# 0xC0000054/avif-format

Hardware: NVIDIA H100
Metric: Gpixels/s (higher is better)
Workload: dtype f32

## Files before the change

avif-format_b200/csrc/kernels_fast_flat.cu:

```cuda
#include "kernels_fast_common.cuh"
#include "table_staging.cuh"
#include "../../include/avifgpu.h"

namespace avifgpu
{

using namespace avifpix;
using namespace fastenc;
using namespace staging;
using avifmath::LibmTables;

namespace
{

#ifndef AVIF_FLAT_WARPS
#define AVIF_FLAT_WARPS 28
#endif
constexpr int kFlatWarps = AVIF_FLAT_WARPS;
constexpr int kFlatThreads = kFlatWarps * 32;
constexpr int kRowSegmentBytes = kTilePixels * 12;
constexpr int kStageBytesPerWarp = 2 * kRowSegmentBytes;
constexpr int kRowSegmentWords = kRowSegmentBytes / 4;
constexpr int kSharedBarriers = 256;
constexpr int kTableBarrierSlot = kSharedBarriers / 8 - 1;
static_assert(kFlatWarps <= kTableBarrierSlot, "the warps' barriers and the table's share kSharedBarriers");
constexpr int kSharedLimit = 227 * 1024;
__host__ __device__ constexpr int FlatFixedBytes() { return kSharedLibm + kSharedBarriers + kFlatWarps * kStageBytesPerWarp; }

struct FlatSchedule
{
    int32_t tilesX, tileRows, warpCount;
    int32_t segments, items;
    int32_t segmentRows, longSegments;
    int32_t lastColumnBytes;
    int32_t unpairedTileRow;
    int32_t scatter;
};

__device__ __forceinline__ bool ElectOne()
{
    uint32_t elected;
    asm volatile("{ .reg .pred p; elect.sync _|p, 0xffffffff; selp.u32 %0, 1, 0, p; }" : "=r"(elected));
    return elected != 0;
}

template <int CURVE, int XS, int YS, int TWO_LEVEL, int INTERLEAVED>
__global__ void __launch_bounds__(kFlatThreads, 1) EncodeRgbF32FlatKernel(const FastEncodeParams p, const FlatSchedule schedule)
{
    constexpr bool kCompact = TWO_LEVEL >= 2;
    constexpr int kCompactShift = TWO_LEVEL == 3 ? 14 : 0;
    extern __shared__ __align__(128) uint8_t sharedBytes[];
    uint64_t* libmStorage = reinterpret_cast<uint64_t*>(sharedBytes);
    uint64_t* barriers = reinterpret_cast<uint64_t*>(sharedBytes + kSharedLibm);
    uint8_t* stageAll = sharedBytes + kSharedLibm + kSharedBarriers;
    uint2* flatEntries = reinterpret_cast<uint2*>(sharedBytes + FlatFixedBytes());
    uint32_t* compactEntries = reinterpret_cast<uint32_t*>(sharedBytes + FlatFixedBytes());
    const uint32_t* firstBits = compactEntries + ((p.table.flatCount + 3) & ~3);
    uint2* octaves = reinterpret_cast<uint2*>(sharedBytes + FlatFixedBytes());
    uint32_t* bucketWords = reinterpret_cast<uint32_t*>(sharedBytes + FlatFixedBytes() + 2048);

    const int lane = threadIdx.x & 31;
    const int warpInBlock = __shfl_sync(0xffffffffu, static_cast<int>(threadIdx.x >> 5), 0);
    const uint32_t barrier = SharedAddress(barriers + warpInBlock);
    uint32_t* stage = reinterpret_cast<uint32_t*>(stageAll + warpInBlock * kStageBytesPerWarp);
    const uint32_t stageAddress = SharedAddress(stage);
    const uint32_t* myStage = stage + lane * 12;

    const int tilesX = schedule.tilesX;
    const int warpCount = schedule.warpCount;
    const int firstItem = schedule.scatter ? warpInBlock * static_cast<int>(gridDim.x) + static_cast<int>(blockIdx.x) : static_cast<int>(blockIdx.x) * kFlatWarps + warpInBlock;
    constexpr int kChromaRowsPerTile = YS ? 1 : 2;
    constexpr int kChromaTileBytes = XS ? kTilePixels : 2 * kTilePixels;

    auto itemRows = [&](int item, int& column, int& rowBegin, int& rowEnd)
    {
        const int segment = item / tilesX;
        column = item - segment * tilesX;
        rowBegin = segment * schedule.segmentRows + min(segment, schedule.longSegments);
        rowEnd = rowBegin + schedule.segmentRows + (segment < schedule.longSegments ? 1 : 0);
    };
    auto fetchTile = [&](int row, uint32_t bytes, int64_t offset)
    {
        const bool second = row != schedule.unpairedTileRow;
        const uint8_t* source = p.rows + offset;
        BarrierExpect(barrier, second ? 2u * bytes : bytes);
        BulkCopyToShared(stageAddress, source, bytes, barrier);
        if (second)
        {
            BulkCopyToShared(stageAddress + kRowSegmentBytes, source + p.rowStride, bytes, barrier);
        }
    };
    auto columnBytes = [&](int column) { return column == tilesX - 1 ? static_cast<uint32_t>(schedule.lastColumnBytes) : static_cast<uint32_t>(kRowSegmentBytes); };
    auto sourceOffsetOf = [&](int row, int column) { return static_cast<int64_t>(row) * 2 * p.rowStride + static_cast<int64_t>(column) * kRowSegmentBytes; };

    if (kCompact && threadIdx.x == 0)
    {
        BeginTableImageCopy(p.table, compactEntries, barriers + kTableBarrierSlot);
    }
    if (ElectOne())
    {
        BarrierInit(barrier, 1);
        BarrierInitFence();
        if (firstItem < schedule.items)
        {
            int column, rowBegin, rowEnd;
            itemRows(firstItem, column, rowBegin, rowEnd);
            if (rowBegin < rowEnd)
            {
                fetchTile(rowBegin, columnBytes(column), sourceOffsetOf(rowBegin, column));
            }
        }
    }

    const LibmTables t = avifmath::StageLibmTables(libmStorage, threadIdx.x, blockDim.x);
    if (kCompact)
    {
    }
    else if (TWO_LEVEL)
    {
        for (int i = threadIdx.x; i < 256; i += blockDim.x)
        {
            octaves[i] = p.table.octaves[i];
        }
        for (int i = threadIdx.x; i < p.table.bucketCount; i += blockDim.x)
        {
            bucketWords[i] = p.table.buckets[i];
        }
    }
    else
    {
        const uint4* source = reinterpret_cast<const uint4*>(p.table.flat);
        uint4* target = reinterpret_cast<uint4*>(flatEntries);
        const int pairs = (p.table.flatCount + 1) / 2;
#pragma unroll 8
        for (int i = threadIdx.x; i < pairs; i += blockDim.x)
        {
            target[i] = __ldg(source + i);
        }
    }
    __syncthreads();
    if (kCompact)
    {
        WaitTableImage(barriers + kTableBarrierSlot);
    }

    const uint32_t flatShift = p.table.flatShift;
    const int32_t negativeLow = -static_cast<int32_t>(p.table.flatLow);
    const int32_t span = static_cast<int32_t>(p.table.flatHigh - p.table.flatLow);
    const uint32_t bandStrideLog2 = p.table.bandStrideLog2;
    const uint32_t* __restrict__ bandBits = p.table.bandBits;
    const uint32_t compactTopShift = 32u - flatShift;
    const uint32_t compactCodeMask = p.table.compactCodeMask;
    const uint32_t compactMagic = p.table.compactMagic;
    uint32_t parity = 0;

#pragma unroll 1
    for (int item = firstItem; item < schedule.items; item += warpCount)
    {
        int column, rowBegin, rowEnd;
        itemRows(item, column, rowBegin, rowEnd);
        if (item != firstItem && rowBegin < rowEnd && ElectOne())
        {
            fetchTile(rowBegin, columnBytes(column), sourceOffsetOf(rowBegin, column));
        }
        const uint32_t tileBytes = columnBytes(column);
        const bool laneActive = column * kTilePixels + lane * 4 < p.width;
        int64_t sourceOffset = sourceOffsetOf(rowBegin, column);
        uint8_t* yPointer = p.planeY + static_cast<int64_t>(rowBegin) * 2 * p.strideY +
                            (INTERLEAVED ? static_cast<int64_t>(column) * (6 * kTilePixels) + lane * 24 : static_cast<int64_t>(column) * (2 * kTilePixels) + lane * 8);
        uint8_t* cbPointer = p.planeCb + static_cast<int64_t>(rowBegin) * kChromaRowsPerTile * p.strideCb + static_cast<int64_t>(column) * kChromaTileBytes + lane * (XS ? 4 : 8);
        uint8_t* crPointer = p.planeCr + static_cast<int64_t>(rowBegin) * kChromaRowsPerTile * p.strideCr + static_cast<int64_t>(column) * kChromaTileBytes + lane * (XS ? 4 : 8);

#pragma unroll 1
    for (int tileRow = rowBegin; tileRow < rowEnd; ++tileRow)
    {
        const bool secondRow = tileRow != schedule.unpairedTileRow;
        sourceOffset += 2 * p.rowStride;

        BarrierWait(barrier, parity);
        parity ^= 1u;

        float codeF[kValuesPerLane];
        uint32_t bandMask = 0;
        int32_t largest = 0;
#pragma unroll
        for (int q = 0; q < 6; ++q)
        {
            const uint4 w = *reinterpret_cast<const uint4*>(myStage + (q / 3) * kRowSegmentWords + (q % 3) * 4);
            const uint32_t bits[4] = { w.x, w.y, w.z, w.w };
#pragma unroll
            for (int e = 0; e < 4; ++e)
            {
                const int j = 4 * q + e;
                bool inBand;
                if (kCompact)
                {
                    uint32_t entry;
                    codeF[j] = LookupCurveCompact<kCompactShift>(bits[e], compactEntries, flatShift, negativeLow, span, compactTopShift, compactCodeMask,
                                                                 compactMagic, inBand, entry);
                }
                else if (TWO_LEVEL)
                {
                    codeF[j] = CodeToFloat(LookupCurveCode(bits[e], octaves, bucketWords, inBand));
                }
                else
                {
                    codeF[j] = LookupCurveFlat(bits[e], flatEntries, flatShift, negativeLow, span, inBand);
                }
                asm("{ .reg .pred p; setp.ne.u32 p, %1, 0; @p or.b32 %0, %0, %2; }" : "+r"(bandMask) : "r"(static_cast<uint32_t>(inBand)), "r"(1u << j));
            }
            if (TWO_LEVEL != 1)
            {
                largest = max(largest, __vimax3_s32(static_cast<int32_t>(w.x), static_cast<int32_t>(w.y), static_cast<int32_t>(w.z)));
                largest = max(largest, static_cast<int32_t>(w.w));
            }
        }

        auto stagedBits = [&](int j) { return myStage[j + (j >= 12 ? kRowSegmentWords - 12 : 0)]; };
        uint32_t lowerMask = 0;
        if (kCompact)
        {
            uint32_t pending = bandMask;
            while (pending != 0)
            {
                uint32_t word[2] = { 0xffffffffu, 0xffffffffu }, index[2] = { 0u, 0u }, sampleBit[2] = { 0u, 0u };
#pragma unroll
                for (int u = 0; u < 2; ++u)
                {
                    if (pending != 0)
                    {
                        const int j = __ffs(static_cast<int>(pending)) - 1;
                        pending &= pending - 1;
                        const uint32_t bits = stagedBits(j);
                        const int32_t bucket = __viaddmin_s32_relu(static_cast<int32_t>(bits) >> flatShift, negativeLow, span);
                        const uint32_t entry = compactEntries[bucket];
                        const uint32_t k = ((entry & compactCodeMask) >> kCompactLenBits) + ((entry >> compactTopShift) != 0 ? 1u : 0u);
                        const uint32_t distance = bits - firstBits[k];
                        if (k != 0 && distance < (1u << bandStrideLog2))
                        {
                            index[u] = (k << bandStrideLog2) + distance;
                            word[u] = __ldg(bandBits + (index[u] >> 5));
                            sampleBit[u] = 1u << j;
                        }
                    }
                }
#pragma unroll
                for (int u = 0; u < 2; ++u)
                {
                    if (((word[u] >> (index[u] & 31u)) & 1u) == 0)
                    {
                        lowerMask |= sampleBit[u];
                    }
                }
            }
        }
        else if (!TWO_LEVEL)
        {
            uint32_t pending = bandMask;
            while (pending != 0)
            {
                const int j0 = __ffs(static_cast<int>(pending)) - 1;
                pending &= pending - 1;
                const uint32_t bits0 = stagedBits(j0);
                bool inBand;
                uint2 entry0;
                LookupCurveFlat(bits0, flatEntries, flatShift, negativeLow, span, inBand, entry0);
                const uint32_t index0 = BandBitIndex(bits0, entry0, bandStrideLog2);
                const uint32_t word0 = __ldg(bandBits + (index0 >> 5));
                uint32_t word1 = 0xffffffffu, index1 = 0, sample1 = 0;
                if (pending != 0)
                {
                    const int j1 = __ffs(static_cast<int>(pending)) - 1;
                    pending &= pending - 1;
                    const uint32_t bits1 = stagedBits(j1);
                    uint2 entry1;
                    LookupCurveFlat(bits1, flatEntries, flatShift, negativeLow, span, inBand, entry1);
                    index1 = BandBitIndex(bits1, entry1, bandStrideLog2);
                    word1 = __ldg(bandBits + (index1 >> 5));
                    sample1 = 1u << j1;
                }
                lowerMask |= (((word0 >> (index0 & 31u)) & 1u) ^ 1u) << j0;
                if (((word1 >> (index1 & 31u)) & 1u) == 0)
                {
                    lowerMask |= sample1;
                }
            }
        }

        if (__any_sync(0xffffffffu, TWO_LEVEL == 1 ? bandMask != 0 : largest > 0x7f7fffff))
        {
            for (int j = 0; j < kValuesPerLane; ++j)
            {
                const uint32_t bits = stagedBits(j);
                if (TWO_LEVEL == 1 ? ((bandMask >> j) & 1u) != 0 : static_cast<int32_t>(bits) > 0x7f7fffff)
                {
                    const float exact = CodeToFloat(ExactCurveCode<CURVE>(__uint_as_float(bits), p.pqMultiplier, p.maxCodeFloat, t));
#pragma unroll
                    for (int slot = 0; slot < kValuesPerLane; ++slot)
                    {
                        if (slot == j)
                        {
                            codeF[slot] = exact;
                        }
                    }
                }
            }
        }

        __syncwarp();
        if (tileRow + 1 < rowEnd && ElectOne())
        {
            fetchTile(tileRow + 1, tileBytes, sourceOffset);
        }

#pragma unroll
        for (int j = 0; j < kValuesPerLane; ++j)
        {
            if (lowerMask & (1u << j))
            {
                codeF[j] -= 1.0f;
            }
        }

        if (laneActive)
        {
            if (INTERLEAVED)
            {
#pragma unroll
                for (int r = 0; r < 2; ++r)
                {
                    if (r == 1 && !secondRow) break;
                    uint32_t words[6];
#pragma unroll
                    for (int w = 0; w < 6; ++w)
                    {
                        words[w] = __float2uint_rz(codeF[12 * r + 2 * w]) | (__float2uint_rz(codeF[12 * r + 2 * w + 1]) << 16);
                    }
                    uint2* target = reinterpret_cast<uint2*>(yPointer + r * p.strideY);
                    __stcs(target, make_uint2(words[0], words[1]));
                    __stcs(target + 1, make_uint2(words[2], words[3]));
                    __stcs(target + 2, make_uint2(words[4], words[5]));
                }
            }
            else
            {
                StoreTile<XS, YS>(p, codeF, yPointer, cbPointer, crPointer, secondRow);
            }
        }
        yPointer += 2 * p.strideY;
        cbPointer += kChromaRowsPerTile * p.strideCb;
        crPointer += kChromaRowsPerTile * p.strideCr;
    }
    }
}

inline size_t TableSharedBytes(const FastEncodeParams& fp, int tableKind)
{
    if (tableKind == 1) return 2048 + static_cast<size_t>(fp.table.bucketCount) * sizeof(uint32_t);
    if (tableKind >= 2) return fp.table.compactImageBytes;
    return static_cast<size_t>((fp.table.flatCount + 1) / 2) * sizeof(uint4);
}

template <int CURVE, int XS, int YS, int TWO_LEVEL, int INTERLEAVED = 0>
cudaError_t LaunchFlatKernel(const FastEncodeParams& fp, int smCount, cudaStream_t stream)
{
    const size_t shared = static_cast<size_t>(FlatFixedBytes()) + TableSharedBytes(fp, TWO_LEVEL);
    static std::atomic<uint64_t> configuredDevices{ 0 };
    {
        const cudaError_t e = AllowDynamicShared(EncodeRgbF32FlatKernel<CURVE, XS, YS, TWO_LEVEL, INTERLEAVED>, kSharedLimit, configuredDevices);
        if (e != cudaSuccess)
        {
            return e;
        }
    }
    const long long tiles = static_cast<long long>((fp.width + kTilePixels - 1) / kTilePixels) * ((fp.rowCount + 1) / 2);
    if (tiles > 0x7fffffffll || shared > static_cast<size_t>(kSharedLimit))
    {
        return cudaErrorInvalidValue;
    }
    long long blocks = (tiles + kFlatWarps - 1) / kFlatWarps;
    if (blocks > smCount)
    {
        blocks = smCount;
    }
    FlatSchedule schedule{};
    schedule.tilesX = (fp.width + kTilePixels - 1) / kTilePixels;
    schedule.tileRows = (fp.rowCount + 1) / 2;
    schedule.warpCount = static_cast<int32_t>(blocks) * kFlatWarps;
    schedule.segments = schedule.warpCount / schedule.tilesX;
    if (schedule.segments < 1) schedule.segments = 1;
    if (schedule.segments > schedule.tileRows) schedule.segments = schedule.tileRows;
    schedule.items = schedule.tilesX * schedule.segments;
    schedule.segmentRows = schedule.tileRows / schedule.segments;
    schedule.longSegments = schedule.tileRows % schedule.segments;
    schedule.lastColumnBytes = (fp.width - (schedule.tilesX - 1) * kTilePixels) * 12;
    schedule.unpairedTileRow = (fp.rowCount & 1) ? fp.rowCount / 2 : -1;
    static const bool scatterOff = []() { const char* v = getenv("AVIFGPU_FLAT_SCATTER"); return v != nullptr && v[0] == '0'; }();
    schedule.scatter = scatterOff ? 0 : 1;
    EncodeRgbF32FlatKernel<CURVE, XS, YS, TWO_LEVEL, INTERLEAVED><<<static_cast<unsigned>(blocks), kFlatThreads, shared, stream>>>(fp, schedule);
    return cudaGetLastError();
}

template <int CURVE, int TWO_LEVEL>
cudaError_t DispatchFlatChroma(const FastEncodeParams& fp, int xs, int ys, int smCount, cudaStream_t stream)
{
    if (xs == 1 && ys == 1) return LaunchFlatKernel<CURVE, 1, 1, TWO_LEVEL>(fp, smCount, stream);
    if (xs == 1) return LaunchFlatKernel<CURVE, 1, 0, TWO_LEVEL>(fp, smCount, stream);
    return LaunchFlatKernel<CURVE, 0, 0, TWO_LEVEL>(fp, smCount, stream);
}

}

static bool FlatTableFits(const FastEncodeParams& fp)
{
    return fp.table.flat != nullptr && fp.table.bandBits != nullptr &&
           static_cast<size_t>(FlatFixedBytes()) + TableSharedBytes(fp, 0) <= static_cast<size_t>(kSharedLimit);
}

static bool CompactTableFits(const FastEncodeParams& fp)
{
    return fp.table.compact != nullptr && fp.table.firstBits != nullptr && fp.table.bandBits != nullptr &&
           static_cast<size_t>(FlatFixedBytes()) + TableSharedBytes(fp, 2) <= static_cast<size_t>(kSharedLimit);
}

static bool TwoLevelTableFits(const FastEncodeParams& fp)
{
    return fp.table.buckets != nullptr && fp.table.octaves != nullptr &&
           static_cast<size_t>(FlatFixedBytes()) + TableSharedBytes(fp, 1) <= static_cast<size_t>(kSharedLimit);
}

bool FlatEncodeApplies(const FastEncodeParams& fp)
{
    return CompactTableFits(fp) || FlatTableFits(fp) || TwoLevelTableFits(fp);
}

cudaError_t LaunchFastEncodeFlatInterleaved(const FastEncodeParams& fp, int curve, int smCount, cudaStream_t stream)
{
    if (CompactTableFits(fp))
    {
        if (curve == kCurveLinearToPQ)
        {
            return fp.table.flatShift == 14 ? LaunchFlatKernel<kCurveLinearToPQ, 0, 0, 3, 1>(fp, smCount, stream) : LaunchFlatKernel<kCurveLinearToPQ, 0, 0, 2, 1>(fp, smCount, stream);
        }
        return LaunchFlatKernel<kCurveLinearToSMPTE428, 0, 0, 2, 1>(fp, smCount, stream);
    }
    if (FlatTableFits(fp))
    {
        if (curve == kCurveLinearToPQ) return LaunchFlatKernel<kCurveLinearToPQ, 0, 0, 0, 1>(fp, smCount, stream);
        return LaunchFlatKernel<kCurveLinearToSMPTE428, 0, 0, 0, 1>(fp, smCount, stream);
    }
    if (curve == kCurveLinearToPQ) return LaunchFlatKernel<kCurveLinearToPQ, 0, 0, 1, 1>(fp, smCount, stream);
    return LaunchFlatKernel<kCurveLinearToSMPTE428, 0, 0, 1, 1>(fp, smCount, stream);
}

cudaError_t LaunchFastEncodeFlat(const FastEncodeParams& fp, int curve, int xs, int ys, int smCount, cudaStream_t stream)
{
    if (CompactTableFits(fp) && !fp.preferWideEntries)
    {
        if (curve == kCurveLinearToPQ)
        {
            return fp.table.flatShift == 14 ? DispatchFlatChroma<kCurveLinearToPQ, 3>(fp, xs, ys, smCount, stream) : DispatchFlatChroma<kCurveLinearToPQ, 2>(fp, xs, ys, smCount, stream);
        }
        return DispatchFlatChroma<kCurveLinearToSMPTE428, 2>(fp, xs, ys, smCount, stream);
    }
    if (FlatTableFits(fp))
    {
        if (curve == kCurveLinearToPQ) return DispatchFlatChroma<kCurveLinearToPQ, 0>(fp, xs, ys, smCount, stream);
        return DispatchFlatChroma<kCurveLinearToSMPTE428, 0>(fp, xs, ys, smCount, stream);
    }
    if (curve == kCurveLinearToPQ) return DispatchFlatChroma<kCurveLinearToPQ, 1>(fp, xs, ys, smCount, stream);
    return DispatchFlatChroma<kCurveLinearToSMPTE428, 1>(fp, xs, ys, smCount, stream);
}

}
```

avif-format_b200/csrc/table_staging.cuh:

```cuda
#ifndef AVIFGPU_TABLE_STAGING_CUH
#define AVIFGPU_TABLE_STAGING_CUH

#include "curve_tables.h"

#include <stdint.h>

namespace avifgpu
{
namespace staging
{

constexpr uint32_t kTableCopyChunk = 16384;

__device__ __forceinline__ uint32_t SharedAddress(const void* pointer) { return static_cast<uint32_t>(__cvta_generic_to_shared(pointer)); }

__device__ __forceinline__ void BarrierInit(uint32_t barrier, uint32_t arrivals)
{
    asm volatile("mbarrier.init.shared::cta.b64 [%0], %1;" ::"r"(barrier), "r"(arrivals) : "memory");
}

__device__ __forceinline__ void BarrierInitFence() { asm volatile("fence.mbarrier_init.release.cluster;" ::: "memory"); }

__device__ __forceinline__ void BarrierExpect(uint32_t barrier, uint32_t bytes)
{
    asm volatile("mbarrier.arrive.expect_tx.shared::cta.b64 _, [%0], %1;" ::"r"(barrier), "r"(bytes) : "memory");
}

__device__ __forceinline__ void BulkCopyToShared(uint32_t target, const void* source, uint32_t bytes, uint32_t barrier)
{
    asm volatile("cp.async.bulk.shared::cluster.global.mbarrier::complete_tx::bytes [%0], [%1], %2, [%3];" ::"r"(target), "l"(source), "r"(bytes),
                 "r"(barrier)
                 : "memory");
}

__device__ __forceinline__ void BarrierWait(uint32_t barrier, uint32_t parity)
{
    asm volatile(
        "{\n"
        ".reg .pred done;\n"
        "WAIT_LOOP:\n"
        "mbarrier.try_wait.parity.shared::cta.b64 done, [%0], %1;\n"
        "@done bra WAIT_DONE;\n"
        "bra WAIT_LOOP;\n"
        "WAIT_DONE:\n"
        "}\n" ::"r"(barrier),
        "r"(parity)
        : "memory");
}

__device__ __forceinline__ void BeginTableImageCopy(const CurveTableView& table, void* sharedImage, uint64_t* barrierStorage)
{
    const uint32_t barrier = SharedAddress(barrierStorage);
    BarrierInit(barrier, 1);
    BarrierInitFence();
    const uint32_t imageBytes = table.compactImageBytes;
    BarrierExpect(barrier, imageBytes);
    const uint32_t target = SharedAddress(sharedImage);
    const uint8_t* source = reinterpret_cast<const uint8_t*>(table.compact);
    for (uint32_t offset = 0; offset < imageBytes; offset += kTableCopyChunk)
    {
        BulkCopyToShared(target + offset, source + offset, min(kTableCopyChunk, imageBytes - offset), barrier);
    }
}

__device__ __forceinline__ void WaitTableImage(uint64_t* barrierStorage) { BarrierWait(SharedAddress(barrierStorage), 0); }

}
}

#endif
```

Measured before the change: 185.8.

## Replace segmented flat schedule with grid-strided tile walk and L2 prefetch

The flat encode kernel no longer splits rows into per-column segments that each warp walks vertically. Each warp now strides through tiles in raster order by the total warp count. It also issues an L2 bulk prefetch for its second tile and loads the compact table with an evict_last cache policy so the table stays resident in L2. The intent is better load balance, interleaved DRAM access across warps and less startup latency, at the cost of losing vertical locality and recomputing output pointers per tile. Profiling probe scripts that compare the encode against copy-throughput ceilings are also added.

```diff
diff --git a/avif-format_b200/csrc/kernels_fast_flat.cu b/avif-format_b200/csrc/kernels_fast_flat.cu
--- a/avif-format_b200/csrc/kernels_fast_flat.cu
+++ b/avif-format_b200/csrc/kernels_fast_flat.cu
@@ -29,12 +29,10 @@
 
 struct FlatSchedule
 {
-    int32_t tilesX, tileRows, warpCount;
-    int32_t segments, items;
-    int32_t segmentRows, longSegments;
+    int32_t tilesX, tileRows;
+    int32_t stepRows, stepColumns;
     int32_t lastColumnBytes;
     int32_t unpairedTileRow;
-    int32_t scatter;
 };
 
 __device__ __forceinline__ bool ElectOne()
@@ -67,22 +65,21 @@
     const uint32_t* myStage = stage + lane * 12;
 
     const int tilesX = schedule.tilesX;
-    const int warpCount = schedule.warpCount;
-    const int firstItem = schedule.scatter ? warpInBlock * static_cast<int>(gridDim.x) + static_cast<int>(blockIdx.x) : static_cast<int>(blockIdx.x) * kFlatWarps + warpInBlock;
+    const int tileRows = schedule.tileRows;
     constexpr int kChromaRowsPerTile = YS ? 1 : 2;
     constexpr int kChromaTileBytes = XS ? kTilePixels : 2 * kTilePixels;
 
-    auto itemRows = [&](int item, int& column, int& rowBegin, int& rowEnd)
-    {
-        const int segment = item / tilesX;
-        column = item - segment * tilesX;
-        rowBegin = segment * schedule.segmentRows + min(segment, schedule.longSegments);
-        rowEnd = rowBegin + schedule.segmentRows + (segment < schedule.longSegments ? 1 : 0);
-    };
-    auto fetchTile = [&](int row, uint32_t bytes, int64_t offset)
+    int tileRow, column;
+    {
+        const int first = warpInBlock * static_cast<int>(gridDim.x) + static_cast<int>(blockIdx.x);
+        tileRow = first / tilesX;
+        column = first - tileRow * tilesX;
+    }
+    auto fetchTile = [&](int row, int col)
     {
         const bool second = row != schedule.unpairedTileRow;
-        const uint8_t* source = p.rows + offset;
+        const uint32_t bytes = col == tilesX - 1 ? static_cast<uint32_t>(schedule.lastColumnBytes) : static_cast<uint32_t>(kRowSegmentBytes);
+        const uint8_t* source = p.rows + static_cast<int64_t>(row) * 2 * p.rowStride + static_cast<int64_t>(col) * kRowSegmentBytes;
         BarrierExpect(barrier, second ? 2u * bytes : bytes);
         BulkCopyToShared(stageAddress, source, bytes, barrier);
         if (second)
@@ -90,25 +87,37 @@
             BulkCopyToShared(stageAddress + kRowSegmentBytes, source + p.rowStride, bytes, barrier);
         }
     };
-    auto columnBytes = [&](int column) { return column == tilesX - 1 ? static_cast<uint32_t>(schedule.lastColumnBytes) : static_cast<uint32_t>(kRowSegmentBytes); };
-    auto sourceOffsetOf = [&](int row, int column) { return static_cast<int64_t>(row) * 2 * p.rowStride + static_cast<int64_t>(column) * kRowSegmentBytes; };
+    auto prefetchSecondTile = [&]()
+    {
+        int row = tileRow + schedule.stepRows, col = column + schedule.stepColumns;
+        if (col >= tilesX)
+        {
+            col -= tilesX;
+            ++row;
+        }
+        if (row < tileRows)
+        {
+            const uint32_t bytes = col == tilesX - 1 ? static_cast<uint32_t>(schedule.lastColumnBytes) : static_cast<uint32_t>(kRowSegmentBytes);
+            const uint8_t* source = p.rows + static_cast<int64_t>(row) * 2 * p.rowStride + static_cast<int64_t>(col) * kRowSegmentBytes;
+            asm volatile("cp.async.bulk.prefetch.L2.global [%0], %1;" ::"l"(source), "r"(bytes) : "memory");
+            if (row != schedule.unpairedTileRow)
+            {
+                asm volatile("cp.async.bulk.prefetch.L2.global [%0], %1;" ::"l"(source + p.rowStride), "r"(bytes) : "memory");
+            }
+        }
+    };
 
     if (kCompact && threadIdx.x == 0)
     {
-        BeginTableImageCopy(p.table, compactEntries, barriers + kTableBarrierSlot);
+        BeginTableImageCopy(p.table, compactEntries, barriers + kTableBarrierSlot, true);
     }
     if (ElectOne())
     {
         BarrierInit(barrier, 1);
         BarrierInitFence();
-        if (firstItem < schedule.items)
-        {
-            int column, rowBegin, rowEnd;
-            itemRows(firstItem, column, rowBegin, rowEnd);
-            if (rowBegin < rowEnd)
-            {
-                fetchTile(rowBegin, columnBytes(column), sourceOffsetOf(rowBegin, column));
-            }
+        if (tileRow < tileRows)
+        {
+            fetchTile(tileRow, column);
         }
     }
 
@@ -142,6 +151,10 @@
     if (kCompact)
     {
         WaitTableImage(barriers + kTableBarrierSlot);
+    }
+    if (tileRow < tileRows && ElectOne())
+    {
+        prefetchSecondTile();
     }
 
     const uint32_t flatShift = p.table.flatShift;
@@ -155,27 +168,15 @@
     uint32_t parity = 0;
 
 #pragma unroll 1
-    for (int item = firstItem; item < schedule.items; item += warpCount)
-    {
-        int column, rowBegin, rowEnd;
-        itemRows(item, column, rowBegin, rowEnd);
-        if (item != firstItem && rowBegin < rowEnd && ElectOne())
-        {
-            fetchTile(rowBegin, columnBytes(column), sourceOffsetOf(rowBegin, column));
-        }
-        const uint32_t tileBytes = columnBytes(column);
-        const bool laneActive = column * kTilePixels + lane * 4 < p.width;
-        int64_t sourceOffset = sourceOffsetOf(rowBegin, column);
-        uint8_t* yPointer = p.planeY + static_cast<int64_t>(rowBegin) * 2 * p.strideY +
-                            (INTERLEAVED ? static_cast<int64_t>(column) * (6 * kTilePixels) + lane * 24 : static_cast<int64_t>(column) * (2 * kTilePixels) + lane * 8);
-        uint8_t* cbPointer = p.planeCb + static_cast<int64_t>(rowBegin) * kChromaRowsPerTile * p.strideCb + static_cast<int64_t>(column) * kChromaTileBytes + lane * (XS ? 4 : 8);
-        uint8_t* crPointer = p.planeCr + static_cast<int64_t>(rowBegin) * kChromaRowsPerTile * p.strideCr + static_cast<int64_t>(column) * kChromaTileBytes + lane * (XS ? 4 : 8);
-
-#pragma unroll 1
-    for (int tileRow = rowBegin; tileRow < rowEnd; ++tileRow)
+    while (tileRow < tileRows)
     {
         const bool secondRow = tileRow != schedule.unpairedTileRow;
-        sourceOffset += 2 * p.rowStride;
+        int nextRow = tileRow + schedule.stepRows, nextColumn = column + schedule.stepColumns;
+        if (nextColumn >= tilesX)
+        {
+            nextColumn -= tilesX;
+            ++nextRow;
+        }
 
         BarrierWait(barrier, parity);
         parity ^= 1u;
@@ -308,9 +309,9 @@
         }
 
         __syncwarp();
-        if (tileRow + 1 < rowEnd && ElectOne())
-        {
-            fetchTile(tileRow + 1, tileBytes, sourceOffset);
+        if (nextRow < tileRows && ElectOne())
+        {
+            fetchTile(nextRow, nextColumn);
         }
 
 #pragma unroll
@@ -322,8 +323,12 @@
             }
         }
 
-        if (laneActive)
-        {
+        if (column * kTilePixels + lane * 4 < p.width)
+        {
+            uint8_t* yPointer = p.planeY + static_cast<int64_t>(tileRow) * 2 * p.strideY +
+                                (INTERLEAVED ? static_cast<int64_t>(column) * (6 * kTilePixels) + lane * 24 : static_cast<int64_t>(column) * (2 * kTilePixels) + lane * 8);
+            uint8_t* cbPointer = p.planeCb + static_cast<int64_t>(tileRow) * kChromaRowsPerTile * p.strideCb + static_cast<int64_t>(column) * kChromaTileBytes + lane * (XS ? 4 : 8);
+            uint8_t* crPointer = p.planeCr + static_cast<int64_t>(tileRow) * kChromaRowsPerTile * p.strideCr + static_cast<int64_t>(column) * kChromaTileBytes + lane * (XS ? 4 : 8);
             if (INTERLEAVED)
             {
 #pragma unroll
@@ -347,10 +352,8 @@
                 StoreTile<XS, YS>(p, codeF, yPointer, cbPointer, crPointer, secondRow);
             }
         }
-        yPointer += 2 * p.strideY;
-        cbPointer += kChromaRowsPerTile * p.strideCb;
-        crPointer += kChromaRowsPerTile * p.strideCr;
-    }
+        tileRow = nextRow;
+        column = nextColumn;
     }
 }
 
@@ -386,17 +389,11 @@
     FlatSchedule schedule{};
     schedule.tilesX = (fp.width + kTilePixels - 1) / kTilePixels;
     schedule.tileRows = (fp.rowCount + 1) / 2;
-    schedule.warpCount = static_cast<int32_t>(blocks) * kFlatWarps;
-    schedule.segments = schedule.warpCount / schedule.tilesX;
-    if (schedule.segments < 1) schedule.segments = 1;
-    if (schedule.segments > schedule.tileRows) schedule.segments = schedule.tileRows;
-    schedule.items = schedule.tilesX * schedule.segments;
-    schedule.segmentRows = schedule.tileRows / schedule.segments;
-    schedule.longSegments = schedule.tileRows % schedule.segments;
+    const int32_t warpCount = static_cast<int32_t>(blocks) * kFlatWarps;
+    schedule.stepRows = warpCount / schedule.tilesX;
+    schedule.stepColumns = warpCount % schedule.tilesX;
     schedule.lastColumnBytes = (fp.width - (schedule.tilesX - 1) * kTilePixels) * 12;
     schedule.unpairedTileRow = (fp.rowCount & 1) ? fp.rowCount / 2 : -1;
-    static const bool scatterOff = []() { const char* v = getenv("AVIFGPU_FLAT_SCATTER"); return v != nullptr && v[0] == '0'; }();
-    schedule.scatter = scatterOff ? 0 : 1;
     EncodeRgbF32FlatKernel<CURVE, XS, YS, TWO_LEVEL, INTERLEAVED><<<static_cast<unsigned>(blocks), kFlatThreads, shared, stream>>>(fp, schedule);
     return cudaGetLastError();
 }
diff --git a/avif-format_b200/csrc/table_staging.cuh b/avif-format_b200/csrc/table_staging.cuh
--- a/avif-format_b200/csrc/table_staging.cuh
+++ b/avif-format_b200/csrc/table_staging.cuh
@@ -33,6 +33,20 @@
                  : "memory");
 }
 
+__device__ __forceinline__ uint64_t PolicyEvictLast()
+{
+    uint64_t policy;
+    asm volatile("createpolicy.fractional.L2::evict_last.b64 %0, 1.0;" : "=l"(policy));
+    return policy;
+}
+
+__device__ __forceinline__ void BulkCopyToShared(uint32_t target, const void* source, uint32_t bytes, uint32_t barrier, uint64_t policy)
+{
+    asm volatile("cp.async.bulk.shared::cluster.global.mbarrier::complete_tx::bytes.L2::cache_hint [%0], [%1], %2, [%3], %4;" ::"r"(target),
+                 "l"(source), "r"(bytes), "r"(barrier), "l"(policy)
+                 : "memory");
+}
+
 __device__ __forceinline__ void BarrierWait(uint32_t barrier, uint32_t parity)
 {
     asm volatile(
@@ -48,7 +62,7 @@
         : "memory");
 }
 
-__device__ __forceinline__ void BeginTableImageCopy(const CurveTableView& table, void* sharedImage, uint64_t* barrierStorage)
+__device__ __forceinline__ void BeginTableImageCopy(const CurveTableView& table, void* sharedImage, uint64_t* barrierStorage, bool keepInL2 = false)
 {
     const uint32_t barrier = SharedAddress(barrierStorage);
     BarrierInit(barrier, 1);
@@ -59,7 +73,15 @@
     const uint8_t* source = reinterpret_cast<const uint8_t*>(table.compact);
     for (uint32_t offset = 0; offset < imageBytes; offset += kTableCopyChunk)
     {
-        BulkCopyToShared(target + offset, source + offset, min(kTableCopyChunk, imageBytes - offset), barrier);
+        const uint32_t bytes = min(kTableCopyChunk, imageBytes - offset);
+        if (keepInL2)
+        {
+            BulkCopyToShared(target + offset, source + offset, bytes, barrier, PolicyEvictLast());
+        }
+        else
+        {
+            BulkCopyToShared(target + offset, source + offset, bytes, barrier);
+        }
     }
 }
 
diff --git a/profiles/c2_ceiling_probe.cu b/profiles/c2_ceiling_probe.cu
--- /dev/null
+++ b/profiles/c2_ceiling_probe.cu
@@ -0,0 +1,138 @@
+#include <cuda_runtime.h>
+#include <stdint.h>
+
+namespace
+{
+
+constexpr int kChunkBytes = 3072;
+constexpr int kChunkOut = kChunkBytes / 4;
+constexpr int kMaxStages = 2;
+
+__device__ __forceinline__ uint4 Xor4(uint4 a, uint4 b, uint4 c, uint4 d)
+{
+    return make_uint4(a.x ^ b.x ^ c.x ^ d.x, a.y ^ b.y ^ c.y ^ d.y, a.z ^ b.z ^ c.z ^ d.z, a.w ^ b.w ^ c.w ^ d.w);
+}
+
+__global__ void __launch_bounds__(256) CopyMixLdg(const uint4* __restrict__ in, uint4* __restrict__ out, long long outWords)
+{
+    const int lane = threadIdx.x & 31;
+    const long long warp = (static_cast<long long>(blockIdx.x) * blockDim.x + threadIdx.x) >> 5;
+    const long long warps = (static_cast<long long>(gridDim.x) * blockDim.x) >> 5;
+    for (long long base = warp * 32; base < outWords; base += warps * 32)
+    {
+        const uint4* source = in + base * 4;
+        const uint4 a = __ldcs(source + lane), b = __ldcs(source + 32 + lane), c = __ldcs(source + 64 + lane), d = __ldcs(source + 96 + lane);
+        __stcs(out + base + lane, Xor4(a, b, c, d));
+    }
+}
+
+__device__ __forceinline__ uint32_t SharedAddress(const void* p) { return static_cast<uint32_t>(__cvta_generic_to_shared(p)); }
+
+__device__ __forceinline__ void Fetch(uint32_t target, const void* source, uint32_t barrier)
+{
+    asm volatile("mbarrier.arrive.expect_tx.shared::cta.b64 _, [%0], %1;" ::"r"(barrier), "r"(kChunkBytes) : "memory");
+    asm volatile("cp.async.bulk.shared::cluster.global.mbarrier::complete_tx::bytes [%0], [%1], %2, [%3];" ::"r"(target), "l"(source),
+                 "r"(kChunkBytes), "r"(barrier)
+                 : "memory");
+}
+
+__device__ __forceinline__ void Wait(uint32_t barrier, uint32_t parity)
+{
+    asm volatile("{\n.reg .pred done;\nPROBE_WAIT:\nmbarrier.try_wait.parity.shared::cta.b64 done, [%0], %1;\n@!done bra PROBE_WAIT;\n}\n" ::"r"(barrier),
+                 "r"(parity)
+                 : "memory");
+}
+
+__global__ void CopyMixBulk(const uint8_t* __restrict__ in, uint4* __restrict__ out, int chunks, int stages)
+{
+    extern __shared__ __align__(128) uint8_t shared[];
+    const int lane = threadIdx.x & 31;
+    const int warpInBlock = __shfl_sync(0xffffffffu, static_cast<int>(threadIdx.x >> 5), 0);
+    const int warpsPerBlock = blockDim.x >> 5;
+    uint64_t* barriers = reinterpret_cast<uint64_t*>(shared) + warpInBlock * kMaxStages;
+    uint8_t* stage = shared + 1024 + warpInBlock * kMaxStages * kChunkBytes;
+    const int warps = warpsPerBlock * gridDim.x;
+    const int first = warpInBlock * gridDim.x + blockIdx.x;
+    if (lane == 0)
+    {
+        for (int s = 0; s < stages; ++s)
+        {
+            asm volatile("mbarrier.init.shared::cta.b64 [%0], 1;" ::"r"(SharedAddress(barriers + s)) : "memory");
+        }
+        asm volatile("fence.mbarrier_init.release.cluster;" ::: "memory");
+        for (int s = 0; s < stages; ++s)
+        {
+            const int chunk = first + s * warps;
+            if (chunk < chunks)
+            {
+                Fetch(SharedAddress(stage + s * kChunkBytes), in + static_cast<long long>(chunk) * kChunkBytes, SharedAddress(barriers + s));
+            }
+        }
+    }
+    __syncwarp();
+    int s = 0;
+    uint32_t parity = 0;
+    for (int chunk = first; chunk < chunks; chunk += warps)
+    {
+        Wait(SharedAddress(barriers + s), parity);
+        const uint4* words = reinterpret_cast<const uint4*>(stage + s * kChunkBytes);
+        uint4* target = out + static_cast<long long>(chunk) * (kChunkOut / 16);
+        const uint4 r0 = Xor4(words[lane], words[32 + lane], words[64 + lane], words[96 + lane]);
+        uint4 r1 = make_uint4(0, 0, 0, 0);
+        if (lane < 16)
+        {
+            r1 = Xor4(words[128 + lane], words[144 + lane], words[160 + lane], words[176 + lane]);
+        }
+        __syncwarp();
+        const int next = chunk + stages * warps;
+        if (lane == 0 && next < chunks)
+        {
+            Fetch(SharedAddress(stage + s * kChunkBytes), in + static_cast<long long>(next) * kChunkBytes, SharedAddress(barriers + s));
+        }
+        __stcs(target + lane, r0);
+        if (lane < 16)
+        {
+            __stcs(target + 32 + lane, r1);
+        }
+        if (++s == stages)
+        {
+            s = 0;
+            parity ^= 1u;
+        }
+    }
+}
+
+}
+
+extern "C" {
+
+int probe_sm_count(int device)
+{
+    int sms = 0;
+    return cudaDeviceGetAttribute(&sms, cudaDevAttrMultiProcessorCount, device) == cudaSuccess ? sms : -1;
+}
+
+int probe_ldg(const void* in, void* out, long long outBytes, int ctasPerSm, int smCount, void* stream)
+{
+    CopyMixLdg<<<ctasPerSm * smCount, 256, 0, static_cast<cudaStream_t>(stream)>>>(static_cast<const uint4*>(in), static_cast<uint4*>(out), outBytes / 16);
+    return static_cast<int>(cudaGetLastError());
+}
+
+int probe_bulk(const void* in, void* out, long long inBytes, int warps, int stages, int smCount, void* stream)
+{
+    if (stages < 1 || stages > kMaxStages || warps < 1 || warps > 32)
+    {
+        return static_cast<int>(cudaErrorInvalidValue);
+    }
+    const int shared = 1024 + warps * kMaxStages * kChunkBytes;
+    cudaError_t e = cudaFuncSetAttribute(CopyMixBulk, cudaFuncAttributeMaxDynamicSharedMemorySize, shared);
+    if (e != cudaSuccess)
+    {
+        return static_cast<int>(e);
+    }
+    CopyMixBulk<<<smCount, warps * 32, shared, static_cast<cudaStream_t>(stream)>>>(static_cast<const uint8_t*>(in), static_cast<uint4*>(out),
+                                                                                  static_cast<int>(inBytes / kChunkBytes), stages);
+    return static_cast<int>(cudaGetLastError());
+}
+
+}
diff --git a/profiles/measure_c2_ceiling.py b/profiles/measure_c2_ceiling.py
--- /dev/null
+++ b/profiles/measure_c2_ceiling.py
@@ -0,0 +1,150 @@
+#!/usr/bin/env python3
+import argparse
+import ctypes as C
+import json
+import os
+import shutil
+import statistics
+import subprocess
+import sys
+import tempfile
+
+HERE = os.path.dirname(os.path.abspath(__file__))
+ROOT = os.path.dirname(HERE)
+
+FRAME_ROWS, HALF_ROWS = 4320, 2160
+
+
+def build_probe(directory):
+    nvcc = shutil.which("nvcc") or "/usr/local/cuda/bin/nvcc"
+    target = os.path.join(directory, "c2_ceiling_probe.so")
+    subprocess.run([nvcc, "-gencode", "arch=compute_90a,code=sm_90a", "-std=c++17", "-O3", "-shared", "-Xcompiler", "-fPIC",
+                    "-o", target, os.path.join(HERE, "c2_ceiling_probe.cu")], check=True, capture_output=True, timeout=600)
+    lib = C.CDLL(target)
+    lib.probe_sm_count.argtypes = [C.c_int]
+    lib.probe_ldg.argtypes = [C.c_void_p, C.c_void_p, C.c_longlong, C.c_int, C.c_int, C.c_void_p]
+    lib.probe_bulk.argtypes = [C.c_void_p, C.c_void_p, C.c_longlong, C.c_int, C.c_int, C.c_int, C.c_void_p]
+    return lib
+
+
+def summary(values):
+    med = statistics.median(values)
+    return {"median": med, "min": min(values), "max": max(values), "spread": (max(values) - min(values)) / med if med else None,
+            "rounds": values}
+
+
+def main():
+    ap = argparse.ArgumentParser()
+    ap.add_argument("--rounds", type=int, default=5)
+    ap.add_argument("--launches", type=int, default=20, help="timed launches per figure per round")
+    ap.add_argument("--out", default=None, help="write the JSON here (it is printed either way)")
+    ap.add_argument("--tree", default=ROOT, help="checkout whose bench.py workload and built library the encode figures use")
+    ap.add_argument("--label", default="this tree")
+    args = ap.parse_args()
+
+    tree = os.path.abspath(args.tree)
+    sys.path.insert(0, tree)
+    import bench
+    import torch
+    import avifgpu
+
+    if not torch.cuda.is_available():
+        raise SystemExit("measure_c2_ceiling.py: no CUDA device")
+    device = torch.device("cuda", 0)
+    torch.cuda.set_device(device)
+    scratch = tempfile.mkdtemp(prefix="c2_ceiling_")
+    try:
+        probe = build_probe(scratch)
+        gpu = avifgpu.Context(0)
+        wl = bench.Workload("c2")
+        run = bench.DeviceRun(torch, avifgpu, gpu, wl, device, 2 * 1000 + 1234)
+        stream = run.stream
+        handle = run.handle
+        in_bytes = wl.w * wl.h * 12
+        out_bytes = in_bytes // 4
+        assert out_bytes == sum(t.numel() * t.element_size() for t in run.outputs[0] if t is not None)
+        probe_out = [torch.empty(out_bytes, dtype=torch.uint8, device=device) for _ in range(run.copies)]
+        sms = torch.cuda.get_device_properties(device).multi_processor_count
+
+        def check(status):
+            if status != 0:
+                raise RuntimeError(f"probe launch failed: cudaError {status}")
+
+        def ldg(ctas_per_sm):
+            return lambda i: check(probe.probe_ldg(run.inputs[i % run.copies][0].data_ptr(), probe_out[i % run.copies].data_ptr(), out_bytes,
+                                                   ctas_per_sm, sms, handle))
+
+        def bulk(warps, stages):
+            return lambda i: check(probe.probe_bulk(run.inputs[i % run.copies][0].data_ptr(), probe_out[i % run.copies].data_ptr(), in_bytes,
+                                                    warps, stages, sms, handle))
+
+        def encode_half(i):
+            rows = run.inputs[i % run.copies][0]
+            gpu.encode_device(wl.enc, rows.data_ptr(), rows.stride(0) * rows.element_size(), avifgpu.planes_from_tensors(run.outputs[i % run.copies]),
+                              y0=0, nrows=HALF_ROWS, stream=handle)
+
+        frame_bytes = in_bytes + out_bytes
+        cases = {}
+        for ctas in (2, 4, 8):
+            cases[f"ldg_{ctas * 8}_warps_per_sm"] = (ldg(ctas), frame_bytes, "copy")
+        for warps in (16, 28):
+            for stages in (1, 2):
+                cases[f"bulk_{warps}_warps_{stages}_buffers"] = (bulk(warps, stages), frame_bytes, "copy")
+        cases["encode_4320_rows"] = (run.launch, wl.algorithmic_bytes, "encode")
+        cases["encode_2160_rows"] = (encode_half, wl.algorithmic_bytes * HALF_ROWS // FRAME_ROWS, "encode")
+
+        for launch, _, _ in cases.values():
+            for i in range(3):
+                launch(i)
+        torch.cuda.synchronize(device)
+
+        per_round = {name: [] for name in cases}
+        back_to_back = {name: [] for name in cases}
+        for _ in range(args.rounds):
+            for name, (launch, _, _) in cases.items():
+                events = [torch.cuda.Event(enable_timing=True) for _ in range(args.launches + 1)]
+                events[0].record(stream)
+                for i in range(args.launches):
+                    launch(i)
+                    events[i + 1].record(stream)
+                torch.cuda.synchronize(device)
+                per = [events[i].elapsed_time(events[i + 1]) for i in range(args.launches)]
+                per_round[name].append(statistics.median(per))
+                back_to_back[name].append(events[0].elapsed_time(events[-1]) / args.launches)
+
+        figures = {}
+        for name, (_, nbytes, kind) in cases.items():
+            ms = summary(per_round[name])
+            figures[name] = {"kind": kind, "bytes_per_launch": nbytes, "launch_ms": ms, "back_to_back_ms": summary(back_to_back[name]),
+                             "tb_s": nbytes / (ms["median"] * 1e-3) / 1e12}
+        copies = {n: f for n, f in figures.items() if f["kind"] == "copy"}
+        best = max(copies, key=lambda n: copies[n]["tb_s"])
+        ceiling = copies[best]["tb_s"]
+        fixed = [2 * h - f for h, f in zip(per_round["encode_2160_rows"], per_round["encode_4320_rows"])]
+        whole = figures["encode_4320_rows"]
+        result = {
+            "what": "config 2 (7680x4320 RGB32f -> 12-bit PQ 4:2:0, 398 MB read + 99.5 MB written) against copy-mix probes of the same traffic",
+            "device": bench.device_identity(torch, 0),
+            "encode_tree": args.label,
+            "environment": {k: v for k, v in os.environ.items() if k.startswith("AVIFGPU_")},
+            "rounds": args.rounds, "launches_per_round": args.launches, "sm_count": sms,
+            "ceiling": {"tb_s": ceiling, "probe": best},
+            "encode": {"tb_s": whole["tb_s"], "frac_of_ceiling": whole["tb_s"] / ceiling, "frac_of_data_sheet": whole["tb_s"] / 3.35,
+                       "gpx_s": wl.pixels / (whole["launch_ms"]["median"] * 1e-3) / 1e9},
+            "fixed_cost_per_launch": {"ms": summary(fixed), "frac_of_frame": statistics.median(fixed) / whole["launch_ms"]["median"],
+                                      "how": "2 t(2160 rows) - t(4320 rows), per round"},
+            "figures": figures,
+        }
+        text = json.dumps(result, indent=1)
+        print(text)
+        if args.out:
+            os.makedirs(os.path.dirname(os.path.abspath(args.out)), exist_ok=True)
+            with open(args.out, "w") as f:
+                f.write(text + "\n")
+        gpu.close()
+    finally:
+        shutil.rmtree(scratch, ignore_errors=True)
+
+
+if __name__ == "__main__":
+    main()
```

Measured after the change: 191.4 (median of 6 runs). +3.0%, better.
